# ossamaAhmed/blackbox_mpc

Measured on AMD Instinct MI355X. Metric: MPC control-steps/sec (agent-control-steps; Pendulum true model, CEM N=500 H=30), higher is better.
Workload: dtype f32; 1 GPU; BASELINE cfg2: Pendulum-v0 true dynamics, CEM, num_agents=1/GPU, N=500, H=30, 5 iters, k=50, closed loop (the model is the environment); parallelism=single GPU

## Files before the change

### blackbox_mpc_amd/csrc/bbmpc.hip

```cpp
#include "engine.hpp"
#include "abi_util.hpp"
#include "engine_util.hpp"
#include "kernels_corr.hpp"
#include "kernels_elite_carry.hpp"

#include <math.h>
#include <stdio.h>
#include <stdlib.h>
#include <atomic>
#include <functional>
#include <chrono>
#include <mutex>
#include <set>
#include <thread>
#include <utility>

namespace bbmpc {

static std::mutex g_engines_mu;
static std::set<Engine*> g_engines;
static std::atomic<int> g_resident_handles{0};
void note_resident_handle() { g_resident_handles.fetch_add(1, std::memory_order_relaxed); }

void stop_foreign_residents(Engine* self) {
// ... 128 lines not shown
        throw HipError(BBMPC_E_NO_DEVICE, "no HIP device available: this library has no CPU fallback");
    if (c.device >= 0) {
        REQUIRE(c.device < ndev, BBMPC_E_NO_DEVICE, "bbmpc_config.device out of range");
        HIP_CHECK(hipSetDevice(c.device));
    }
    HIP_CHECK(hipGetDevice(&device));
    HIP_CHECK(hipDeviceGetAttribute(&cu_count, hipDeviceAttributeMultiprocessorCount, device));
    {
        int least = 0, greatest = 0;
        HIP_CHECK(hipDeviceGetStreamPriorityRange(&least, &greatest));
        if (!(own_stream = masked_stream_from_env("BBMPC_STREAM_CUS", cu_count)))
            HIP_CHECK(hipStreamCreateWithPriority(&own_stream, hipStreamNonBlocking, greatest));
    }
    stream = own_stream;
    init_tnq_table();

    if (const char* fm = getenv("BBMPC_FUSED")) fused_mode = atoi(fm);
    {
        auto flag = [](const char* n) { return getenv(n) != nullptr; };
        auto ival = [](const char* n, int dflt) { const char* v = getenv(n); return v ? atoi(v) : dflt; };
        sw.cma_svd_v1 = flag("BBMPC_CMA_SVD_V1"); sw.cma_svd_rounds = flag("BBMPC_CMA_SVD_ROUNDS");
        sw.cma_svd_general = flag("BBMPC_CMA_SVD_GENERAL");
        sw.cma_svd_gram = flag("BBMPC_CMA_SVD_GRAM");
        sw.cma_coop = flag("BBMPC_CMA_COOP"); sw.cma_nb = ival("BBMPC_CMA_NB", 0);
        sw.cma_eigh = ival("BBMPC_CMA_EIGH", 1); sw.cma_eigh_fail = flag("BBMPC_CMA_EIGH_FAIL");
        sw.cma_fused = flag("BBMPC_CMA_FUSED");
        sw.mlp_generic = flag("BBMPC_MLP_GENERIC");
        { const int b = ival("BBMPC_MLP_BF16", 0); sw.mlp_bf16 = (b == 1 || b == 3) ? b : 0; }
        sw.mlp_pair = ival("BBMPC_MLP_PAIR", -1); sw.mlp_q4 = ival("BBMPC_MLP_Q4", -1); sw.mlp_q4s = ival("BBMPC_MLP_Q4S", ival("BBMPC_MLP_Q4R", 1)); sw.mlp_w4 = ival("BBMPC_MLP_W4", 1); sw.pi2_skip_init = ival("BBMPC_PI2_SKIP_INIT", 1); sw.step_graph = ival("BBMPC_STEP_GRAPH", 1); sw.cma_small3 = ival("BBMPC_CMA_SMALL3", 1);
        sw.refit_wgs = ival("BBMPC_REFIT_WGS", 0);
        sw.mlp_wave = ival("BBMPC_MLP_WAVE", 1);
        sw.linger_us = std::max(0, ival("BBMPC_LINGER_US", 200));
        linger_test_quit = ival("BBMPC_LINGER_TEST_QUIT", 0) - 1;
        sw.balance = ival("BBMPC_BALANCE", 0);
        sw.ilp = ival("BBMPC_ILP", 1) == 2 ? 2 : 1;
        sw.refit_v1 = flag("BBMPC_REFIT_V1");
        sw.zero_copy = !flag("BBMPC_NO_ZERO_COPY");
        sw.host_poll = !flag("BBMPC_NO_HOST_POLL");
        sw.mlp_no_half_tail = flag("BBMPC_MLP_NO_HALF_TAIL");
        sw.dbg = flag("BBMPC_DBG");
        sw.prof_reward_mlp = flag("BBMPC_PROF_REWARD_MLP");
        user_stepwise_only = flag("BBMPC_USER_STEPWISE");
        if (c.optimizer != BBMPC_OPT_NONE) {
            ps_loopback = auto_split > 1 ? auto_split : ival("BBMPC_POPSHARD_LOOPBACK", 0);
            ps_force = flag("BBMPC_POPSHARD_FORCE");
        }
    }
    HU = H * U;
    Nst = ((std::max(N, 1) + 63) / 64) * 64;
    rec = U + S + 1;
    lo.assign(c.action_low, c.action_low + U);
    hi.assign(c.action_high, c.action_high + U);
    upload(d_lo, lo);
    upload(d_hi, hi);
    d_state.alloc((size_t)A * S);
    d_record.alloc((size_t)A * rec);
    d_action.alloc((size_t)A * U);
    d_action.zero(stream);
    if (c.optimizer != BBMPC_OPT_NONE) {
        std::vector<float> m((size_t)A * HU), v((size_t)A * HU);
        for (int i = 0; i < A * HU; ++i) {
            const int u = i % U;
            m[i] = (lo[u] + hi[u]) / 2.0f;
            const float d = lo[u] - hi[u];
            v[i] = (d * d) / 16.0f;
        }
// ... 45 lines not shown
    }
    if (pf_stream) {
        (void)hipStreamSynchronize(pf_stream);
        (void)hipStreamDestroy(pf_stream);
        for (int b = 0; b < 2; ++b)
            if (pf_done[b]) (void)hipEventDestroy(pf_done[b]);
        if (pf_free) (void)hipEventDestroy(pf_free);
    }
    for (auto e : ev_pool) (void)hipEventDestroy(e);
    user_reward.release();
    user_dynamics.release();
    user_rollout.release();
    user_xform.release();
    user_fwd_xform.release();
    user_xform_rollout.release();
    if (h_pin) (void)hipHostFree(h_pin);
    for (auto*& hs : h_record_stage) { if (hs) (void)hipHostFree(hs); hs = nullptr; }
    if (host_done) (void)hipHostFree(host_done);
    if (host_count) (void)hipFree(host_count);
    if (own_stream) (void)hipStreamDestroy(own_stream);
}

void Engine::settle() {
    if (settle_hook) settle_hook(this);
    resident_stop();
    if (lazy_sync) {
        lazy_sync = false;
        HIP_CHECK(hipStreamSynchronize(stream));
    }
}

static void resident_unpublish(Engine* e);

bool Engine::resident_step(const float* state, int add_noise, uint32_t seq) {
    {
        bool all_gone = true;
        for (int a = 0; a < A && all_gone; ++a) all_gone = *(volatile const uint32_t*)gone_host(a) != 0u;
        if (all_gone) {
            resident_unpublish(this);
            resident_alive = false;
            return false;
        }
    }
    const uint32_t step = step_counter;
    const int64_t c = (int64_t)step / std::max(pf_steps, 1);
    const int pb = (int)(c & 1), nb = pb ^ 1;
    if (pf_mode != 1 || pf_chunk[pb] != c) { resident_stop(); return false; }
    if (!pf_waited[pb]) {
        if (hipEventQuery(pf_done[pb]) != hipSuccess) { resident_stop(); return false; }
        pf_waited[pb] = true; pf_inflight[pb] = false;
    }
    const float* inj = d_noise_pf[pb].p + (size_t)((int64_t)step - c * pf_steps) * pf_step_floats;
    ++step_counter;
    const uint64_t ip = (uint64_t)(uintptr_t)inj;
    for (int a = 0; a < A; ++a) {
        volatile uint32_t* m = mbox_host(a);
        uint32_t sw3[3];
        memcpy(sw3, state + (size_t)a * 3, 12);
        const uint32_t tag = seq & 0xffffu;
        const uint16_t half[13] = {(uint16_t)step, (uint16_t)(step >> 16), (uint16_t)(add_noise != 0),
                                   (uint16_t)ip, (uint16_t)(ip >> 16), (uint16_t)(ip >> 32), (uint16_t)(ip >> 48),
                                   (uint16_t)sw3[0], (uint16_t)(sw3[0] >> 16), (uint16_t)sw3[1], (uint16_t)(sw3[1] >> 16),
                                   (uint16_t)sw3[2], (uint16_t)(sw3[2] >> 16)};
        for (int i = 0; i < 13; ++i) m[i] = ((uint32_t)half[i] << 16) | tag;
        m[15] = seq;
    }
    std::atomic_thread_fence(std::memory_order_release);
    if (pf_chunk[nb] != c + 1) {
        launch_noise_fill(c + 1, nb, pf_stream);
        HIP_CHECK(hipEventRecord(pf_done[nb], pf_stream));
        pf_chunk[nb] = c + 1; pf_waited[nb] = false; pf_inflight[nb] = true;
    }
    if (in_flight_hook && !in_flight_called) { in_flight_called = true; in_flight_hook(this); }
    const auto t0 = std::chrono::steady_clock::now();
    bool all = true;
    for (int a = 0; a < A; ++a) {
        volatile const uint32_t* ack = ack_host(a);
        volatile const uint32_t* gone = gone_host(a);
        uint32_t spins = 0;
        for (;;) {
            if (*ack == seq) break;
            if (*gone != 0u) { all = false; break; }
            if ((++spins & 0xfff) == 0 && std::chrono::steady_clock::now() - t0 > std::chrono::seconds(2)) { all = false; break; }
        }
    }
    if (all) return true;
    resident_stop();
    int missing = 0;
    int32_t* amap = amap_host();
    for (int a = 0; a < A; ++a)
        if (*(volatile const uint32_t*)ack_host(a) != seq) amap[missing++] = a;
    if (missing == 0) return true;
    --step_counter;
    subset_n = missing < A ? missing : 0;
    return false;
}

static void resident_unpublish(Engine* e) {
    if (e->mbox_pub.load(std::memory_order_relaxed)) {
        e->mbox_pub.store(nullptr, std::memory_order_release);
        g_resident_handles.fetch_sub(1, std::memory_order_relaxed);
    }
}

void Engine::resident_stop() {
    if (!resident_alive) return;
    resident_unpublish(this);
    for (int a = 0; a < A; ++a) mbox_host(a)[15] = 0xffffffffu;
    std::atomic_thread_fence(std::memory_order_release);
    resident_alive = false;
    HIP_CHECK(hipStreamSynchronize(stream));
}

float* Engine::pinned(size_t count) {
    if (count > h_pin_n) {
        invalidate_step_graph();
        if (h_pin) (void)hipHostFree(h_pin);
        h_pin = nullptr;
        h_pin_n = 0;
        HIP_CHECK(hipHostMalloc((void**)&h_pin, count * sizeof(float), hipHostMallocCoherent | hipHostMallocMapped));
        h_pin_n = count;
        HIP_CHECK(hipHostGetDevicePointer((void**)&h_pin_dev, h_pin, 0));
    }
    return h_pin;
// ... 1223 lines not shown

}

static const float* optimize_host(bbmpc::Engine& e, const float* state, int32_t noise, float* action, float* next_state, float* reward) {
    using namespace bbmpc;
    const size_t ns = (size_t)e.A * e.S, nr = (size_t)e.A * e.rec;
    float* pin = e.pinned(ns + nr);
    memcpy(pin, state, ns * 4);
    bool published = false;
    bool handled_resident = false;
    const bool fused_step = e.sw.zero_copy && (e.use_fused() || e.use_fused_pso());
    const bool mlp_tail = e.sw.zero_copy && !fused_step && e.cfg.optimizer != BBMPC_OPT_NONE;
    if (fused_step || mlp_tail) {
        float* dpin = e.h_pin_dev;
        if (e.sw.host_poll && !e.trace_on) {
            if (!e.host_done) {
                HIP_CHECK(hipHostMalloc((void**)&e.host_done, (size_t)e.sync_lines() * 64, hipHostMallocCoherent | hipHostMallocMapped));
                memset(e.host_done, 0, (size_t)e.sync_lines() * 64);
                HIP_CHECK(hipHostGetDevicePointer((void**)&e.host_done_dev, e.host_done, 0));
                HIP_CHECK(hipMalloc((void**)&e.host_count, 8));
                HIP_CHECK(hipMemset(e.host_count, 0, 8));
            }
            if (++e.host_seq == 0) e.host_seq = 1;
            e.tail_flag = e.host_done_dev;
            e.tail_count = e.host_count;
            e.tail_value = e.host_seq;
            e.tail_attached = false;
        }
        const bool linger_ok = fused_step && e.tail_flag != nullptr && e.sw.linger_us > 0 && e.A <= Engine::kLingerMaxAgents && e.use_fused() &&
                               !e.profiling && e.tail_event == nullptr &&
                               e.stream == e.own_stream;
        bool handled = false;
        if (e.resident_alive) {
            if (linger_ok) handled = e.resident_step(pin, noise, e.host_seq);
            else e.resident_stop();
        }
        if (handled) ++e.calls_resident; else ++e.calls_launched;
        if (handled) {
            published = true;
            handled_resident = true;
            e.tail_flag = nullptr;
        } else
        try {
            e.linger_launch = linger_ok && e.subset_n == 0;
            if (fused_step) {
                e.optimize_dev(dpin, noise, dpin + ns, nullptr);
            } else {
                const bool stage = (e.cfg.optimizer == BBMPC_OPT_CEM || e.cfg.optimizer == BBMPC_OPT_PI2) && !e.pop_sharded() &&
                                   !e.user_path() && !e.value_on();
                const bool graph_ok = e.sw.step_graph && stage && e.cfg.dynamics == BBMPC_DYN_MLP && e.tail_flag != nullptr &&
                                      e.tail_event == nullptr && !e.profiling && !e.trace_on && !e.particles_on() && !e.corr_on() && !e.carry_on() && e.stream == e.own_stream && !e.any_injected();
                const uint64_t sig = ((uint64_t)e.mutations << 8) | (uint64_t)(noise ? 1 : 0) | 2u;
                bool replayed = false;
                if (graph_ok && e.step_graph && e.step_graph_sig == sig) {
                    replayed = true;
                } else if (graph_ok && e.step_graph_warm >= 3 && e.step_warm_sig == sig) {
                    if (e.step_graph) { (void)hipGraphExecDestroy(e.step_graph); e.step_graph = nullptr; }
                    if (!e.step_words) {
                        HIP_CHECK(hipHostMalloc((void**)&e.step_words, 64, 0));
                        memset(e.step_words, 0, 64);
                        HIP_CHECK(hipMalloc((void**)&e.step_words_dev, 64));
                        HIP_CHECK(hipMemset(e.step_words_dev, 0, 64));
                        e.step_mirror[0] = e.step_mirror[1] = 0xFFFFFFFFu;
                    }
                    const uint32_t saved_step = e.step_counter;
                    hipGraph_t g = nullptr;
                    bool ok = hipStreamBeginCapture(e.stream, hipStreamCaptureModeThreadLocal) == hipSuccess;
// ... 36 lines not shown
                e.optimize_dev(e.d_state.p, noise, dpin + ns, nullptr);
                if (e.stage_state_src) {
                    e.stage_state_src = nullptr;
                    throw HipError(BBMPC_E_HIP, "internal: the control step did not stage its state");
                }
                if (graph_ok && e.last_step_steady && e.step_warm_sig == sig) ++e.step_graph_warm;
                else { e.step_graph_warm = (graph_ok && e.last_step_steady) ? 1 : 0; e.step_warm_sig = sig; }
                }
            }
            e.linger_launch = false;
            published = e.tail_flag != nullptr && e.tail_attached;
            e.tail_flag = nullptr;
        } catch (...) {
            e.linger_launch = false;
            e.tail_flag = nullptr;
            e.subset_n = 0;
            throw;
        }
    } else {
        ++e.calls_launched;
        HIP_CHECK(hipMemcpyAsync(e.d_state.p, pin, ns * 4, hipMemcpyHostToDevice, e.stream));
        e.optimize_dev(e.d_state.p, noise, e.d_record.p, nullptr);
        HIP_CHECK(hipMemcpyAsync(pin + ns, e.d_record.p, nr * 4, hipMemcpyDeviceToHost, e.stream));
    }
    if (e.in_flight_hook && !e.in_flight_called) { e.in_flight_called = true; e.in_flight_hook(&e); }
    if (handled_resident) {
        std::atomic_thread_fence(std::memory_order_acquire);
        e.lazy_sync = true;
    } else if (published && e.resident_alive) {
        const uint32_t want = e.host_seq;
        const auto t0 = std::chrono::steady_clock::now();
        for (int a = 0; a < e.A; ++a) {
            volatile const uint32_t* f = e.ack_host(a);
            uint32_t spins = 0;
            while (*f != want) {
                if ((++spins & 0xfff) == 0 && std::chrono::steady_clock::now() - t0 > std::chrono::seconds(2)) {
                    e.resident_stop();
                    if (*f != want) throw HipError(BBMPC_E_HIP, "bbmpc_optimize: the control step finished without publishing its records");
                }
            }
        }
        std::atomic_thread_fence(std::memory_order_acquire);
        e.lazy_sync = true;
    } else if (published) {
        volatile const uint32_t* f = e.host_done;
        const uint32_t want = e.host_seq;
        const auto t0 = std::chrono::steady_clock::now();
        uint32_t spins = 0;
        while (*f != want) {
            if ((++spins & 0xfff) == 0 && std::chrono::steady_clock::now() - t0 > std::chrono::seconds(2)) {
                HIP_CHECK(hipStreamSynchronize(e.stream));
                if (*f != want) throw HipError(BBMPC_E_HIP, "bbmpc_optimize: the control step finished without publishing its records");
                break;
            }
        }
        std::atomic_thread_fence(std::memory_order_acquire);
        e.lazy_sync = true;
    } else {
        HIP_CHECK(hipStreamSynchronize(e.stream));
        e.lazy_sync = false;
    }
    const float* r = pin + ns;
    for (int a = 0; a < e.A; ++a) {
        if (action) memcpy(action + (size_t)a * e.U, r + (size_t)a * e.rec, e.U * 4);
        if (next_state) memcpy(next_state + (size_t)a * e.S, r + (size_t)a * e.rec + e.U, e.S * 4);
        if (reward) reward[a] = r[(size_t)a * e.rec + e.U + e.S];
    }
    return r;
}

extern "C" {
// ... 552 lines not shown
```

### blackbox_mpc_amd/csrc/bbmpc_fused.hip

```cpp
#define BBMPC_TU_FUSED
#include "engine.hpp"
#include "engine_util.hpp"

#include <atomic>
#include <chrono>

namespace bbmpc {

void bbmpc_tu_fused_upload_tnq(const float2* table) { tnq_upload(table); }

bool Engine::use_fused() const {
    if (cfg.dynamics != BBMPC_DYN_PENDULUM || cfg.reward != BBMPC_REW_PENDULUM) return false;
    if (pop_sharded()) return false;
    if (particles_on()) return false;
    if (corr_on()) return false;
    if (carry_on()) return false;
    if (cfg.optimizer == BBMPC_OPT_SPSA) {
        if (iters > FUSED_MAX_SPSA_ITERS) return false;
    } else if (cfg.optimizer != BBMPC_OPT_RANDOM_SEARCH && cfg.optimizer != BBMPC_OPT_CEM && cfg.optimizer != BBMPC_OPT_PI2) {
        return false;
    }
    if (fused_mode == 0) return false;
    if (fused_mode == 1) return true;
    return (long)N <= 2048 || A >= 64;
}

static void note_inst(Engine& e, int opt, bool samples_lds, bool fastm, int inj, int ilp, bool linger) {
    snprintf(e.dominant_inst, sizeof(e.dominant_inst), "k_fused_pendulum<%d, %s, %s, %d, %d, %s>", opt, samples_lds ? "true" : "false",
             fastm ? "true" : "false", inj, ilp, linger ? "true" : "false");
}

template <int OPT, bool FASTM, int INJ, int ILP>
static void launch_fused4(Engine& e, FusedArgs& fa, int threads, size_t lds_base, size_t lds_samples) {
#ifdef BBMPC_KERNEL_DBG
    const size_t limit = 158 * 1024;
#else
    const size_t limit = 160 * 1024;
#endif
    if (lds_base + lds_samples <= limit) {
        fa.test_quit_agent = -1;
        if constexpr (INJ == 2 && FASTM && ILP == 1) {
            if (e.linger_launch && e.subset_n == 0 && fa.done_flag && e.tail_event == nullptr) {
                auto fl = k_fused_pendulum<OPT, true, FASTM, INJ, ILP, true>;
                note_inst(e, OPT, true, FASTM, INJ, ILP, true);
                ensure_max_lds((const void*)fl, (int)limit);
                for (int a = 0; a < e.A; ++a) {
                    volatile uint32_t* m = e.mbox_host(a);
                    for (int i = 0; i < 13; ++i) m[i] = fa.done_value & 0xffffu;
                    m[15] = fa.done_value;
                    *(volatile uint32_t*)e.gone_host(a) = 0u;
                }
                std::atomic_thread_fence(std::memory_order_release);
                fa.done_flag = e.sync_dev(e.ack_host(0));
                fa.mbox = e.sync_dev(e.mbox_host(0));
                fa.gone = e.sync_dev(e.gone_host(0));
                fa.linger_ticks = (unsigned)e.sw.linger_us * 100u;
                fa.test_quit_agent = e.linger_test_quit;
                hipLaunchKernelGGL(fl, dim3(e.A), dim3(threads), lds_base + lds_samples, e.stream, fa);
                HIP_CHECK(hipGetLastError());
                e.resident_alive = true;
                if (!e.mbox_pub.load(std::memory_order_relaxed)) {
                    e.mbox_pub_agents = e.A;
                    e.mbox_pub.store(e.mbox_host(0), std::memory_order_release);
                    note_resident_handle();
                }
                return;
            }
        }
        if (e.subset_n > 0) {
            auto fs = k_fused_pendulum<OPT, true, FASTM, INJ, ILP>;
            note_inst(e, OPT, true, FASTM, INJ, ILP, false);
            ensure_max_lds((const void*)fs, (int)limit);
            fa.amap = reinterpret_cast<const int*>(e.sync_dev(e.amap_host()));
            hipLaunchKernelGGL(fs, dim3(e.subset_n), dim3(threads), lds_base + lds_samples, e.stream, fa);
            HIP_CHECK(hipGetLastError());
            e.subset_n = 0;
            return;
        }
        auto fn = k_fused_pendulum<OPT, true, FASTM, INJ, ILP>;
        note_inst(e, OPT, true, FASTM, INJ, ILP, false);
        ensure_max_lds((const void*)fn, (int)limit);
// ... 76 lines not shown
    fa.inj_expl = injected(BBMPC_NOISE_EXPLORATION);
    if (cfg.optimizer == BBMPC_OPT_SPSA) {
        const float big_a = (float)iters / 10.0f;
        for (int it = 0; it < iters && it < FUSED_MAX_SPSA_ITERS; ++it) {
            const float tf = (float)it;
            fa.spsa_ak[it] = cfg.spsa_a / (float)pow((double)((tf + 1.0f) + big_a), (double)cfg.spsa_alpha);
            fa.spsa_ck[it] = cfg.spsa_c / (float)pow((double)(tf + 1.0f), (double)cfg.spsa_gamma);
        }
    }
    fa.record = d_record_out;
    fa.next_state = d_next_out;
    if (trace_on) {
        ensure_trace();
        fa.t_rewards = t_rewards.p; fa.t_mean = t_mean.p; fa.t_var = t_var.p; fa.t_elites = t_elites.p; fa.t_samples = t_samples.p;
        if (cfg.optimizer == BBMPC_OPT_SPSA) {
            if (!t_rewards2.p) t_rewards2.alloc((size_t)A * Nst * std::max(iters, 1));
            fa.t_rewards2 = t_rewards2.p;
        }
    }
#ifdef BBMPC_KERNEL_DBG
    static long long* dbg_buf = nullptr;
    if (sw.dbg) {
        if (!dbg_buf) {
            HIP_CHECK(hipHostMalloc((void**)&dbg_buf, 64 * 8, hipHostMallocDefault));
            memset(dbg_buf, 0, 64 * 8);
        }
        if (dbg_buf[42]) {
            const long long* d = dbg_buf;
            fprintf(stderr, "[dbg] last resident pass, 10ns units rel. to its start:");
            for (int i = 0; i <= 1 + iters * 4; ++i) fprintf(stderr, " %lld", d[i] - d[0]);
            fprintf(stderr, "\n[dbg] iter0 per-wave rollout end:");
            for (int i = 24; i < 32; ++i) fprintf(stderr, " %lld", d[i] - d[0]);
            fprintf(stderr, "\n[dbg] request accepted %lld  first model step %lld  completion stored %lld\n", d[42] - d[0], d[44] - d[0], d[43] - d[0]);
            dbg_buf[42] = 0;
        }
        fa.dbg = dbg_buf;
    }
#endif
    fa.key = key(step);
    const int pf_nit = cfg.optimizer == BBMPC_OPT_RANDOM_SEARCH ? 1 : iters;
    if (pf_mode < 0) {
        const char* ev = getenv("BBMPC_NOISE_PREFETCH");
        pf_step_floats = (size_t)pf_nit * A * Nst * ((HU + 3) / 4) * 4;
        const size_t budget = (size_t)128 << 20;
        pf_steps = pf_step_floats ? (int)std::min<size_t>(8, budget / (pf_step_floats * 4)) : 0;
        pf_mode = ((ev ? atoi(ev) != 0 : true) && pf_steps >= 1 && U == 1) ? 1 : 0;
        if (pf_mode) {
            {
                int least = 0, greatest = 0;
                HIP_CHECK(hipDeviceGetStreamPriorityRange(&least, &greatest));
                HIP_CHECK(hipStreamCreateWithPriority(&pf_stream, hipStreamNonBlocking, greatest));
            }
            HIP_CHECK(hipEventCreateWithFlags(&pf_free, hipEventDisableTiming));
            for (int b = 0; b < 2; ++b) {
                d_noise_pf[b].alloc(pf_step_floats * pf_steps);
                HIP_CHECK(hipEventCreateWithFlags(&pf_done[b], hipEventDisableTiming));
            }
        }
    }
    const bool use_pf = pf_mode == 1 && fa.inj == nullptr && pf_nit > 0;
    if (use_pf) {
        const int64_t c = (int64_t)step / pf_steps;
        const int pb = (int)(c & 1), nb = pb ^ 1;
        if (pf_chunk[pb] != c) {
            if (pf_inflight[pb]) HIP_CHECK(hipStreamWaitEvent(stream, pf_done[pb], 0));
            launch_noise_fill(c, pb, stream);
// ... 117 lines not shown
```

### blackbox_mpc_amd/csrc/engine.hpp

```cpp
#pragma once
#include <hip/hip_ext.h>
#include <hip/hip_runtime.h>
#include <stdint.h>
#include <string.h>

#include <algorithm>
#include <atomic>
#include <map>
#include <stdexcept>
#include <string>
#include <vector>

#include "../../include/bbmpc.h"
#include "comm.hpp"
#include "kernels_cma.hpp"
#include "kernels_eigh.hpp"
#include "kernels_eigh_small.hpp"
#include "kernels_fused.hpp"
#include "kernels_fused_cma.hpp"
#include "kernels_fused_pso.hpp"
#include "kernels_mlp.hpp"
#include "kernels_mlp_xform.hpp"
#include "kernels_mlp_q4s.hpp"
#include "kernels_mlp_w4.hpp"
#include "kernels_mlp_wave.hpp"
#include "kernels_opt.hpp"
#include "kernels_refit.hpp"
#include "kernels_reward_mlp.hpp"
#include "kernels_rollout.hpp"
#include "kernels_tail.hpp"
#include "kernels_user.hpp"

namespace bbmpc {

struct ParticleArgs;
struct TrajParticleArgs;

struct HipError : std::runtime_error {
    int code;
    HipError(int c, const std::string& m) : std::runtime_error(m), code(c) {}
};

#define HIP_CHECK(expr)                                                                          \
    do {                                                                                         \
        hipError_t _e = (expr);                                                                  \
        if (_e != hipSuccess)                                                                    \
            throw HipError(BBMPC_E_HIP, std::string(#expr) + " failed: " + hipGetErrorString(_e) + \
// ... 151 lines not shown
    float* gather_deferred_dst[RecordComm::kSlots] = {nullptr, nullptr};
    void (*settle_hook)(Engine*) = nullptr;
    void (*in_flight_hook)(Engine*) = nullptr;
    bool in_flight_called = false;
    hipEvent_t tail_event = nullptr;
    bool tail_attached = false;
    uint32_t* tail_flag = nullptr;
    uint32_t tail_value = 0;
    uint32_t* tail_count = nullptr;
    uint32_t* host_done = nullptr;
    uint32_t* host_done_dev = nullptr;
    uint32_t* host_count = nullptr;
    uint32_t host_seq = 0;
    bool lazy_sync = false;
    void settle();
    const float* stage_state_src = nullptr;
    bool linger_launch = false;
    bool resident_alive = false;
    static constexpr int kLingerMaxAgents = 64;
    int sync_lines() const {
        const int al = std::max(1, std::min(A, kLingerMaxAgents));
        return 1 + 3 * al + (al + 15) / 16;
    }
    uint32_t* ack_host(int a) { return host_done + 16 * (1 + a); }
    uint32_t* mbox_host(int a) { return host_done + 16 * (1 + std::min(A, kLingerMaxAgents) + a); }
    uint32_t* gone_host(int a) { return host_done + 16 * (1 + 2 * std::min(A, kLingerMaxAgents) + a); }
    int32_t* amap_host() { return reinterpret_cast<int32_t*>(host_done + 16 * (1 + 3 * std::min(A, kLingerMaxAgents))); }
    uint32_t* sync_dev(const void* host_ptr) { return host_done_dev + (reinterpret_cast<const uint32_t*>(host_ptr) - host_done); }
    std::atomic<uint32_t*> mbox_pub{nullptr};
    int mbox_pub_agents = 0;
    int subset_n = 0;
    int linger_test_quit = -1;
    int64_t calls_resident = 0, calls_launched = 0;
    bool resident_step(const float* state, int add_noise, uint32_t seq);
    void resident_stop();
    hipStream_t pf_stream = nullptr;
    hipEvent_t pf_done[2] = {nullptr, nullptr}, pf_free = nullptr;
    int64_t pf_chunk[2] = {-1, -1};
    bool pf_waited[2] = {false, false}, pf_inflight[2] = {false, false};
    int pf_steps = 0;
    size_t pf_step_floats = 0;
    int pf_mode = -1;
    void launch_noise_fill(int64_t chunk, int buf, hipStream_t on);
    std::vector<hipEvent_t> ev_pool;
    size_t ev_used = 0;
    const char* dominant_kernel = "k_rollout_pendulum";
    char dominant_inst[128] = "";

    explicit Engine(const bbmpc_config& c);
    ~Engine();

    RngKey key(uint32_t step) const {
        RngKey kk;
        kk.k0 = (uint32_t)(cfg.seed & 0xffffffffu);
        kk.k1 = (uint32_t)(cfg.seed >> 32);
        kk.step = step;
        kk.q_per_agent = (uint32_t)((HU + 3) / 4);
        kk.step_src = step_capturing ? step_words_dev : nullptr;
        return kk;
    }
    bool fix(uint32_t bit) const { return (cfg.quirks & bit) != 0; }
    UserFunction user_reward, user_dynamics, user_rollout;
    bool user_rollout_stale = true;
    bool user_stepwise_only = false;
    void rollout_user_fused(int mode, bool pen, RolloutArgs& ra);
    void rollout_mlp_user_reward(int mode, bool pen, RolloutArgs& ra);
    DevBuf<float> u_traj;
// ... 209 lines not shown
```

### blackbox_mpc_amd/csrc/kernels_fused.hpp

```cpp
#pragma once
#include <type_traits>

#include "kernels_opt.hpp"
#include "kernels_refit.hpp"
#include "kernels_rollout.hpp"
#include "topk.hpp"

namespace bbmpc {

constexpr int FOPT_RS = 1;
constexpr int FOPT_CEM = 2;
constexpr int FOPT_PI2 = 3;
constexpr int FOPT_SPSA = 4;
constexpr int FUSED_MAX_SPSA_ITERS = 16;

struct FusedArgs {
    int N, A, H, U, HU, Nst, k, iters;
    int agent_offset;
    int fix_q1, fix_q7, add_noise;
    int warm_start;
    int balance;
    unsigned* done_flag;
    unsigned* done_count;
    unsigned done_value;
// ... 96 lines not shown
                mean[tid] = m_keep;
                var[tid] = v_keep;
                sigma[tid] = (OPT == FOPT_CEM && p.warm_start) ? cem_sigma(m_keep, v_keep, lo, hi) : s_keep;
            }
        } else {
            for (int j = tid; j < p.HU; j += nthr) {
                const float m = p.prev_mean[a * p.HU + j];
                const float v = p.var0[a * p.HU + j];
                const float sg = (OPT == FOPT_CEM) ? cem_sigma(m, v, lo, hi) : ((OPT == FOPT_SPSA) ? 0.0f : sqrtf(v));
                mean[j] = m;
                var[j] = v;
                sigma[j] = sg;
                if (keep_init) { m_keep = m; v_keep = v; s_keep = sg; }
            }
        }
    };
    typedef float pfvec4 __attribute__((ext_vector_type(4)));
    typedef const __attribute__((address_space(1))) pfvec4* pfvec4p;
    [[maybe_unused]] pfvec4 pf0 = {0.0f, 0.0f, 0.0f, 0.0f}, pf1 = {0.0f, 0.0f, 0.0f, 0.0f};
    [[maybe_unused]] auto prefetch_first = [&](const float* base, int it_n) {
        if constexpr (INJ == 2) {
            const int Q = (p.HU + 3) >> 2;
            if (tid < p.N) {
                const pfvec4p q = (pfvec4p)(reinterpret_cast<const float4*>(base) + noise_block_index(it_n, p.A, a, p.Nst, tid, Q));
                pf0 = q[0];
                if (OPT != FOPT_SPSA) pf1 = q[min(1, Q - 1)];
            }
        }
    };
    dist_init(false);
    __syncthreads();
    float s0 = red[60], s1 = red[61], s2 = red[62];
    if (p.iters > 0) prefetch_first(inj_s, 0);
    for (;;) {

        float action0 = (OPT == FOPT_RS) ? 0.0f : mean[0];

        BB_DBG(0);
#ifdef BBMPC_KERNEL_DBG
        if (p.dbg && tid == 0 && a == 0) dbg_lds[40] = (long long)clock64();
#endif
        for (int it = 0; it < p.iters; ++it) {
            BB_DBG(1 + it * 4);
            const float* inj = (INJ == 1) ? inj_s + ((size_t)it * p.A + a) * p.HU * p.Nst : nullptr;
            const int nblk = p.H >> 2, rem = p.H & 3;
            const uint32_t rstream = (OPT == FOPT_RS) ? 2u : 1u;
            auto with_q1 = [&](auto&& body) {
                if constexpr (FASTM) {
                    if (p.fix_q1 != 0) { body(std::true_type{}); return; }
                }
                body(std::false_type{});
            };
            if constexpr (OPT == FOPT_SPSA) {
                const float ck = p.spsa_ck[it];
                const int nb4 = (p.H + 3) >> 2;
                with_q1([&](auto Q1c) {
                constexpr bool Q1 = decltype(Q1c)::value;
                for (int n = tid; n < p.N; n += nthr) {
                    Roller<FASTM> rp, rm;
                    rp.init(p.fix_q1 != 0, s0, s1, s2);
                    rm.init(p.fix_q1 != 0, s0, s1, s2);
                    float tp = 0.0f, tm = 0.0f, pp = 0.0f, pm = 0.0f;
                    typedef float gvec4s __attribute__((ext_vector_type(4)));
                    typedef const __attribute__((address_space(1))) gvec4s* gvec4sp;
                    [[maybe_unused]] gvec4sp mine4 = nullptr;
                    [[maybe_unused]] gvec4s cur4 = {1.0f, 1.0f, 1.0f, 1.0f};
// ... 344 lines not shown
                }
                __syncthreads();
                action0 = mean[0];
            } else {
                float bv = -INFINITY;
                int bi = 0x7fffffff;
                for (int n = tid; n < p.N; n += nthr) {
                    const float v = rew[n];
                    if (v > bv || (v == bv && n < bi)) { bv = v; bi = n; }
                }
                wave_argmax(bv, bi);
                int* redi = (int*)(red + 32);
                if ((tid & 63) == 0) { red[tid >> 6] = bv; redi[tid >> 6] = bi; }
                __syncthreads();
                bv = ((tid & 63) < nw) ? red[tid & 63] : -INFINITY;
                bi = ((tid & 63) < nw) ? redi[tid & 63] : 0x7fffffff;
                wave_argmax(bv, bi);
                if (bi == 0x7fffffff) bi = 0;
                action0 = samp[bi];
                if (p.t_elites && tid == 0) p.t_elites[a] = bi;
                __syncthreads();
            }
            if (p.t_mean && OPT != FOPT_RS)
                for (int j = tid; j < p.HU; j += nthr) {
                    p.t_mean[((size_t)it * p.A + a) * p.HU + j] = mean[j];
                    p.t_var[((size_t)it * p.A + a) * p.HU + j] = var[j];
                }
        }

        BB_DBG(1 + p.iters * 4);
#ifdef BBMPC_KERNEL_DBG
        if (p.dbg && tid == 0 && a == 0) dbg_lds[41] = (long long)clock64();
#endif
        if (OPT != FOPT_RS) {
            for (int j = tid; j < p.HU; j += nthr) {
                p.mean_out[a * p.HU + j] = mean[j];
                p.var_out[a * p.HU + j] = var[j];
                if (OPT == FOPT_PI2 || OPT == FOPT_SPSA) {
                    const int js = (j + 1 < p.HU) ? j + 1 : p.HU - 1;
                    const float pm = mean[js];
                    p.prev_mean[a * p.HU + j] = pm;
                    if (keep_init) m_keep = pm;
                } else if (p.warm_start) {
                    const float pm = mean[j];
                    p.prev_mean[a * p.HU + j] = pm;
                    if (keep_init) m_keep = pm;
                }
            }
        }

        if (tid == 0) {
            FinalArgs fa;
            fa.A = p.A; fa.U = 1; fa.S = 3;
            fa.agent_offset = p.agent_offset;
            fa.fix_q1 = p.fix_q1; fa.fix_q7 = p.fix_q7;
            fa.add_noise = add_noise_s;
            fa.lo = p.lo; fa.hi = p.hi;
            fa.inj = p.inj_expl;
            fa.key = key_s;
            fa.key.q_per_agent = 1;
            float s[3] = {s0, s1, s2};
            float act[1];
            act[0] = exploration_action(fa, a, 0, action0);
            const float r = model.step(s, act);
            float* rec = p.record + (size_t)a * 5;
            rec[0] = act[0];
            rec[1] = s[0];
            rec[2] = s[1];
            rec[3] = s[2];
            rec[4] = r;
            if (p.next_state) {
                p.next_state[a * 3 + 0] = s[0];
                p.next_state[a * 3 + 1] = s[1];
                p.next_state[a * 3 + 2] = s[2];
            }
            if constexpr (LINGER) publish_records_done(p.done_flag + a * 16, nullptr, done_value_s, 1u);
            else publish_records_done(p.done_flag, p.done_count, done_value_s, gridDim.x);
            BB_DBG(43);
#ifdef BBMPC_KERNEL_DBG
            if (p.dbg && a == 0) for (int i = 0; i < 48; ++i) p.dbg[i] = dbg_lds[i];
#endif
        }
        if constexpr (!LINGER) {
            break;
        } else {
            unsigned* mb = (unsigned*)ekeys;
            __syncthreads();
            dist_init(keep_init);
            [[maybe_unused]] const float* inj_pred = nullptr;
            if constexpr (INJ == 2) {
                if (p.pf_step_floats)
                    for (int b = 0; b < 2; ++b)
                        if (inj_s >= p.pf_buf[b] && inj_s + 2 * p.pf_step_floats <= p.pf_buf[b] + p.pf_chunk_floats) inj_pred = inj_s + p.pf_step_floats;
                if (inj_pred && p.iters > 0) prefetch_first(inj_pred, 0);
            }
            if (tid < 64) {
                const long long t0 = (long long)wall_clock64();
                const unsigned want = done_value_s + 1u;
                unsigned w = 0u;
                bool quit = false;
                for (;;) {
                    w = (tid < 16) ? __hip_atomic_load(p.mbox + a * 16 + tid, __ATOMIC_RELAXED, __HIP_MEMORY_SCOPE_SYSTEM) : 0u;
                    const bool mine = tid < 13 ? (w & 0xffffu) == (want & 0xffffu) : (tid == 15 ? w == want : true);
                    const unsigned w15 = __builtin_amdgcn_readlane(w, 15);
                    if (__builtin_amdgcn_ballot_w64(mine) == ~0ull) break;
                    if (w15 == 0xffffffffu || (long long)wall_clock64() - t0 > (long long)p.linger_ticks || a == p.test_quit_agent || (p.test_quit_agent >= 999 && a >= p.test_quit_agent - 999)) { quit = true; break; }
                }
                if (tid < 16) mb[tid] = (quit && tid == 15) ? 0xffffffffu : w;
                BB_DBG(42);
            }
            __syncthreads();
            if (mb[15] == 0xffffffffu) {
                if (tid == 0) __hip_atomic_store(p.gone + a * 16, done_value_s, __ATOMIC_RELEASE, __HIP_MEMORY_SCOPE_SYSTEM);
                return;
            }
// ... 15 lines not shown
```

### blackbox_mpc_amd/csrc/kernels_refit.hpp

```cpp
#pragma once
#include <hip/hip_runtime.h>
#include <math.h>
#include "models.hpp"
#include "rng.hpp"
#include "topk.hpp"

namespace bbmpc {

constexpr int REFIT_THREADS = 1024;

#define BB_DPP_QUAD_XOR1 0xB1
#define BB_DPP_QUAD_XOR2 0x4E
#define BB_DPP_ROW_HALF_MIRROR 0x141
#define BB_DPP_ROW_MIRROR 0x140
#define BB_DPP_ROW_SHR(n) (0x110 + (n))

template <int CTRL>
__device__ __forceinline__ float dpp_f(float v) {
    return __int_as_float(__builtin_amdgcn_update_dpp(0, __float_as_int(v), CTRL, 0xf, 0xf, false));
}
template <int CTRL>
__device__ __forceinline__ int dpp_i(int v) {
    return __builtin_amdgcn_update_dpp(0, v, CTRL, 0xf, 0xf, false);
}
// ... 277 lines not shown
}

static __global__ void k_argmax_merge(RefitArgs p, const float* all, int G) {
    const int a = blockIdx.x, lane = threadIdx.x;
    const size_t pw = (size_t)p.A * (p.U + 2);
    int br = 0, bi = 0x7fffffff;
    float bv = -INFINITY;
    for (int r = 0; r < G; ++r) {
        const float* e = all + pw * r + (size_t)a * (p.U + 2);
        const float v = e[0];
        const int idx = __float_as_int(e[1]);
        if (v > bv || (v == bv && idx < bi) || bi == 0x7fffffff) { bv = v; bi = idx; br = r; }
    }
    const float* src = all + pw * br + (size_t)a * (p.U + 2) + 2;
    if (lane == 0 && p.elites) p.elites[a] = bi;
    if (lane < p.U) p.action[a * p.U + lane] = src[lane];
}

struct FinalArgs {
    int A, U, S;
    int agent_offset;
    int fix_q1, fix_q7;
    int add_noise;
    const float* state;
    const float* action;
    const float* lo;
    const float* hi;
    const float* inj;
    float* record;
    float* next_state;
    RngKey key;
};

__device__ __forceinline__ float exploration_action(const FinalArgs& p, int a, int u, float act) {
    if (!p.add_noise) return act;
    float xi;
    if (p.inj) xi = p.inj[a * p.U + u];
    else {
        U4 b = rng_block(rng_key_now(p.key), 10u , 0u, 0u, (uint32_t)(p.agent_offset + a), (uint32_t)u);
        xi = word_to_trunc_normal(pick_word(b, (uint32_t)u));
    }
    const float lo = p.lo[u], hi = p.hi[u];
    const float d = lo - hi;
    const float var = (d * d) / 16.0f * 0.05f;
    const float mean = p.fix_q7 ? 0.0f : (hi + lo) / 2.0f;
    const float noise = xi * sqrtf(var) + mean;
    return clipf(act + noise, lo, hi);
}

__device__ __forceinline__ void finalize_pendulum_agent(const FinalArgs& p, int a, float action_in) {
    const PendulumModel model{p.fix_q1 != 0};
    float s[3] = {p.state[a * 3 + 0], p.state[a * 3 + 1], p.state[a * 3 + 2]};
    float act[1];
    act[0] = exploration_action(p, a, 0, action_in);
    const float r = model.step(s, act);
    float* rec = p.record + (size_t)a * (1 + 3 + 1);
    rec[0] = act[0];
    rec[1] = s[0];
    rec[2] = s[1];
    rec[3] = s[2];
    rec[4] = r;
    if (p.next_state) {
        p.next_state[a * 3 + 0] = s[0];
        p.next_state[a * 3 + 1] = s[1];
        p.next_state[a * 3 + 2] = s[2];
    }
}
__device__ __forceinline__ void publish_records_done(unsigned* flag, unsigned* count, unsigned value, unsigned nwg) {
    if (!flag) return;
    if (nwg == 1u) {
        __hip_atomic_store(flag, value, __ATOMIC_RELEASE, __HIP_MEMORY_SCOPE_SYSTEM);
        return;
    }
    const unsigned old = __hip_atomic_fetch_add(count, 1u, __ATOMIC_RELEASE, __HIP_MEMORY_SCOPE_AGENT);
    if (old == nwg - 1u) {
        __builtin_amdgcn_fence(__ATOMIC_ACQUIRE, "agent");
        __hip_atomic_store(count, 0u, __ATOMIC_RELAXED, __HIP_MEMORY_SCOPE_AGENT);
        __hip_atomic_store(flag, value, __ATOMIC_RELEASE, __HIP_MEMORY_SCOPE_SYSTEM);
    }
}
// ... 12 lines not shown
```

Baseline: 29980 control-steps/s.

## Publish pendulum step record inside the completion line and move tail earlier

The resident (lingering) pendulum kernel now packs the 5-float step record into the 64-byte completion line. Each 32-bit word carries 16 record bits plus a 16-bit sequence tag, written by 16 lanes with system-scope atomic stores. The host decodes the record straight from that line while polling, avoiding a separate record write and its fence-ordered publish. The tail (noise, model step, publish) also runs before the mean/carry stores, to cut latency to the host. This adds tag-based torn-read detection and an encoding constraint that the record is exactly 5 floats.

Result: faster. 30530 control-steps/s, median of 6 (+1.8%).

```diff
diff --git a/blackbox_mpc_amd/csrc/bbmpc.hip b/blackbox_mpc_amd/csrc/bbmpc.hip
--- a/blackbox_mpc_amd/csrc/bbmpc.hip
+++ b/blackbox_mpc_amd/csrc/bbmpc.hip
@@ -184,6 +184,7 @@
         sw.mlp_wave = ival("BBMPC_MLP_WAVE", 1);
         sw.linger_us = std::max(0, ival("BBMPC_LINGER_US", 200));
         linger_test_quit = ival("BBMPC_LINGER_TEST_QUIT", 0) - 1;
+        host_seq = (uint32_t)ival("BBMPC_TEST_HOST_SEQ", 0);
         sw.balance = ival("BBMPC_BALANCE", 0);
         sw.ilp = ival("BBMPC_ILP", 1) == 2 ? 2 : 1;
         sw.refit_v1 = flag("BBMPC_REFIT_V1");
@@ -295,7 +296,7 @@
 
 static void resident_unpublish(Engine* e);
 
-bool Engine::resident_step(const float* state, int add_noise, uint32_t seq) {
+bool Engine::resident_step(const float* state, int add_noise, uint32_t seq, float* records) {
     {
         bool all_gone = true;
         for (int a = 0; a < A && all_gone; ++a) all_gone = *(volatile const uint32_t*)gone_host(a) != 0u;
@@ -342,7 +343,7 @@
         volatile const uint32_t* gone = gone_host(a);
         uint32_t spins = 0;
         for (;;) {
-            if (*ack == seq) break;
+            if (completion_line_decode(ack, seq, records + (size_t)a * kCompletionRecordFloats)) break;
             if (*gone != 0u) { all = false; break; }
             if ((++spins & 0xfff) == 0 && std::chrono::steady_clock::now() - t0 > std::chrono::seconds(2)) { all = false; break; }
         }
@@ -352,7 +353,7 @@
     int missing = 0;
     int32_t* amap = amap_host();
     for (int a = 0; a < A; ++a)
-        if (*(volatile const uint32_t*)ack_host(a) != seq) amap[missing++] = a;
+        if (!completion_line_decode(ack_host(a), seq, records + (size_t)a * kCompletionRecordFloats)) amap[missing++] = a;
     if (missing == 0) return true;
     --step_counter;
     subset_n = missing < A ? missing : 0;
@@ -1642,7 +1643,7 @@
                                e.stream == e.own_stream;
         bool handled = false;
         if (e.resident_alive) {
-            if (linger_ok) handled = e.resident_step(pin, noise, e.host_seq);
+            if (linger_ok) handled = e.resident_step(pin, noise, e.host_seq, pin + ns);
             else e.resident_stop();
         }
         if (handled) ++e.calls_resident; else ++e.calls_launched;
@@ -1745,11 +1746,12 @@
         const auto t0 = std::chrono::steady_clock::now();
         for (int a = 0; a < e.A; ++a) {
             volatile const uint32_t* f = e.ack_host(a);
+            float* rec_a = pin + ns + (size_t)a * kCompletionRecordFloats;
             uint32_t spins = 0;
-            while (*f != want) {
+            while (!completion_line_decode(f, want, rec_a)) {
                 if ((++spins & 0xfff) == 0 && std::chrono::steady_clock::now() - t0 > std::chrono::seconds(2)) {
                     e.resident_stop();
-                    if (*f != want) throw HipError(BBMPC_E_HIP, "bbmpc_optimize: the control step finished without publishing its records");
+                    if (!completion_line_decode(f, want, rec_a)) throw HipError(BBMPC_E_HIP, "bbmpc_optimize: the control step finished without publishing its records");
                 }
             }
         }
diff --git a/blackbox_mpc_amd/csrc/bbmpc_fused.hip b/blackbox_mpc_amd/csrc/bbmpc_fused.hip
--- a/blackbox_mpc_amd/csrc/bbmpc_fused.hip
+++ b/blackbox_mpc_amd/csrc/bbmpc_fused.hip
@@ -44,9 +44,11 @@
                 auto fl = k_fused_pendulum<OPT, true, FASTM, INJ, ILP, true>;
                 note_inst(e, OPT, true, FASTM, INJ, ILP, true);
                 ensure_max_lds((const void*)fl, (int)limit);
+                if (e.rec != kCompletionRecordFloats) throw HipError(BBMPC_E_HIP, "internal: the resident pendulum kernel's record is not 5 floats");
                 for (int a = 0; a < e.A; ++a) {
                     volatile uint32_t* m = e.mbox_host(a);
-                    for (int i = 0; i < 13; ++i) m[i] = fa.done_value & 0xffffu;
+                    volatile uint32_t* cl = e.ack_host(a);
+                    for (int i = 0; i < 16; ++i) cl[i] = (fa.done_value - 1u) & 0xffffu;                    for (int i = 0; i < 13; ++i) m[i] = fa.done_value & 0xffffu;
                     m[15] = fa.done_value;
                     *(volatile uint32_t*)e.gone_host(a) = 0u;
                 }
@@ -189,6 +191,9 @@
             fprintf(stderr, "\n[dbg] iter0 per-wave rollout end:");
             for (int i = 24; i < 32; ++i) fprintf(stderr, " %lld", d[i] - d[0]);
             fprintf(stderr, "\n[dbg] request accepted %lld  first model step %lld  completion stored %lld\n", d[42] - d[0], d[44] - d[0], d[43] - d[0]);
+            const long long sel = d[iters > 0 ? 4 * iters : 0];
+            fprintf(stderr, "[dbg] tail rel. to the last selection: tail start %lld  noise applied %lld  model step %lld  record stored %lld  published %lld  last barrier %lld  carry stored %lld\n",
+                    d[38] - sel, d[35] - sel, d[36] - sel, d[37] - sel, d[43] - sel, d[1 + iters * 4] - sel, d[34] - sel);
             dbg_buf[42] = 0;
         }
         fa.dbg = dbg_buf;
diff --git a/blackbox_mpc_amd/csrc/completion_line.hpp b/blackbox_mpc_amd/csrc/completion_line.hpp
--- /dev/null
+++ b/blackbox_mpc_amd/csrc/completion_line.hpp
@@ -0,0 +1,35 @@
+#pragma once
+#include <cstdint>
+#include <cstring>
+
+namespace bbmpc {
+
+constexpr int kCompletionRecordFloats = 5;
+
+inline bool completion_line_decode(const volatile uint32_t* line, uint32_t seq, float* rec) {
+    if (line[15] != seq) return false;
+    uint32_t w[2 * kCompletionRecordFloats];
+    for (int i = 0; i < 2 * kCompletionRecordFloats; ++i) w[i] = line[i];
+    const uint32_t tag = seq & 0xffffu;
+    for (int i = 0; i < 2 * kCompletionRecordFloats; ++i)
+        if ((w[i] & 0xffffu) != tag) return false;
+    for (int f = 0; f < kCompletionRecordFloats; ++f) {
+        const uint32_t bits = (w[2 * f] >> 16) | (w[2 * f + 1] & 0xffff0000u);
+        memcpy(rec + f, &bits, 4);
+    }
+    return true;
+}
+
+inline void completion_line_encode(uint32_t* line, uint32_t seq, const float* rec) {
+    const uint32_t tag = seq & 0xffffu;
+    for (int f = 0; f < kCompletionRecordFloats; ++f) {
+        uint32_t bits;
+        memcpy(&bits, rec + f, 4);
+        line[2 * f] = (bits << 16) | tag;
+        line[2 * f + 1] = (bits & 0xffff0000u) | tag;
+    }
+    for (int i = 2 * kCompletionRecordFloats; i < 15; ++i) line[i] = tag;
+    line[15] = seq;
+}
+
+}
diff --git a/blackbox_mpc_amd/csrc/engine.hpp b/blackbox_mpc_amd/csrc/engine.hpp
--- a/blackbox_mpc_amd/csrc/engine.hpp
+++ b/blackbox_mpc_amd/csrc/engine.hpp
@@ -13,6 +13,7 @@
 
 #include "../../include/bbmpc.h"
 #include "comm.hpp"
+#include "completion_line.hpp"
 #include "kernels_cma.hpp"
 #include "kernels_eigh.hpp"
 #include "kernels_eigh_small.hpp"
@@ -230,7 +231,7 @@
     int subset_n = 0;
     int linger_test_quit = -1;
     int64_t calls_resident = 0, calls_launched = 0;
-    bool resident_step(const float* state, int add_noise, uint32_t seq);
+    bool resident_step(const float* state, int add_noise, uint32_t seq, float* records);
     void resident_stop();
     hipStream_t pf_stream = nullptr;
     hipEvent_t pf_done[2] = {nullptr, nullptr}, pf_free = nullptr;
diff --git a/blackbox_mpc_amd/csrc/kernels_fused.hpp b/blackbox_mpc_amd/csrc/kernels_fused.hpp
--- a/blackbox_mpc_amd/csrc/kernels_fused.hpp
+++ b/blackbox_mpc_amd/csrc/kernels_fused.hpp
@@ -152,6 +152,53 @@
     __syncthreads();
     float s0 = red[60], s1 = red[61], s2 = red[62];
     if (p.iters > 0) prefetch_first(inj_s, 0);
+    auto noise_term = [&]() {
+        FinalArgs fa;
+        fa.A = p.A; fa.U = 1; fa.S = 3;
+        fa.agent_offset = p.agent_offset;
+        fa.fix_q1 = p.fix_q1; fa.fix_q7 = p.fix_q7;
+        fa.add_noise = add_noise_s;
+        fa.lo = p.lo; fa.hi = p.hi;
+        fa.inj = p.inj_expl;
+        fa.key = key_s;
+        fa.key.q_per_agent = 1;
+        return exploration_noise(fa, a, 0, lo, hi);
+    };
+    const bool tail_lanes = LINGER ? tid < 64 : tid == 0;
+    auto tail = [&](float act_in) {
+        BB_DBG(38);
+        float s[3] = {s0, s1, s2};
+        float act[1];
+        act[0] = add_noise_s ? exploration_apply(act_in, noise_term(), lo, hi) : act_in;
+        BB_DBG(35);
+        const float r = model.step(s, act);
+        BB_DBG(36);
+        if constexpr (LINGER) {
+            const unsigned tag = done_value_s & 0xffffu;
+            const float f = tid < 2 ? act[0] : (tid < 4 ? s[0] : (tid < 6 ? s[1] : (tid < 8 ? s[2] : r)));
+            const unsigned bits = __float_as_uint(f);
+            unsigned w = ((tid & 1) ? (bits & 0xffff0000u) : (bits << 16)) | tag;
+            if (tid >= 10) w = tag;
+            if (tid == 15) w = done_value_s;
+            if (tid < 16) __hip_atomic_store(p.done_flag + a * 16 + tid, w, __ATOMIC_RELAXED, __HIP_MEMORY_SCOPE_SYSTEM);
+            BB_DBG(37);
+        } else {
+            float* rec = p.record + (size_t)a * 5;
+            rec[0] = act[0];
+            rec[1] = s[0];
+            rec[2] = s[1];
+            rec[3] = s[2];
+            rec[4] = r;
+            if (p.next_state) {
+                p.next_state[a * 3 + 0] = s[0];
+                p.next_state[a * 3 + 1] = s[1];
+                p.next_state[a * 3 + 2] = s[2];
+            }
+            BB_DBG(37);
+            publish_records_done(p.done_flag, p.done_count, done_value_s, gridDim.x);
+        }
+        BB_DBG(43);
+    };
     for (;;) {
 
         float action0 = (OPT == FOPT_RS) ? 0.0f : mean[0];
@@ -562,6 +609,7 @@
 #ifdef BBMPC_KERNEL_DBG
         if (p.dbg && tid == 0 && a == 0) dbg_lds[41] = (long long)clock64();
 #endif
+        if (tail_lanes) tail(action0);
         if (OPT != FOPT_RS) {
             for (int j = tid; j < p.HU; j += nthr) {
                 p.mean_out[a * p.HU + j] = mean[j];
@@ -578,39 +626,10 @@
                 }
             }
         }
-
-        if (tid == 0) {
-            FinalArgs fa;
-            fa.A = p.A; fa.U = 1; fa.S = 3;
-            fa.agent_offset = p.agent_offset;
-            fa.fix_q1 = p.fix_q1; fa.fix_q7 = p.fix_q7;
-            fa.add_noise = add_noise_s;
-            fa.lo = p.lo; fa.hi = p.hi;
-            fa.inj = p.inj_expl;
-            fa.key = key_s;
-            fa.key.q_per_agent = 1;
-            float s[3] = {s0, s1, s2};
-            float act[1];
-            act[0] = exploration_action(fa, a, 0, action0);
-            const float r = model.step(s, act);
-            float* rec = p.record + (size_t)a * 5;
-            rec[0] = act[0];
-            rec[1] = s[0];
-            rec[2] = s[1];
-            rec[3] = s[2];
-            rec[4] = r;
-            if (p.next_state) {
-                p.next_state[a * 3 + 0] = s[0];
-                p.next_state[a * 3 + 1] = s[1];
-                p.next_state[a * 3 + 2] = s[2];
-            }
-            if constexpr (LINGER) publish_records_done(p.done_flag + a * 16, nullptr, done_value_s, 1u);
-            else publish_records_done(p.done_flag, p.done_count, done_value_s, gridDim.x);
-            BB_DBG(43);
-#ifdef BBMPC_KERNEL_DBG
-            if (p.dbg && a == 0) for (int i = 0; i < 48; ++i) p.dbg[i] = dbg_lds[i];
-#endif
-        }
+        BB_DBG(34);
+#ifdef BBMPC_KERNEL_DBG
+        if (p.dbg && a == 0 && tid == 0) for (int i = 0; i < 48; ++i) p.dbg[i] = dbg_lds[i];
+#endif
         if constexpr (!LINGER) {
             break;
         } else {
diff --git a/blackbox_mpc_amd/csrc/kernels_refit.hpp b/blackbox_mpc_amd/csrc/kernels_refit.hpp
--- a/blackbox_mpc_amd/csrc/kernels_refit.hpp
+++ b/blackbox_mpc_amd/csrc/kernels_refit.hpp
@@ -333,20 +333,25 @@
     RngKey key;
 };
 
-__device__ __forceinline__ float exploration_action(const FinalArgs& p, int a, int u, float act) {
-    if (!p.add_noise) return act;
+__device__ __forceinline__ float exploration_noise(const FinalArgs& p, int a, int u, float lo, float hi) {
     float xi;
     if (p.inj) xi = p.inj[a * p.U + u];
     else {
         U4 b = rng_block(rng_key_now(p.key), 10u , 0u, 0u, (uint32_t)(p.agent_offset + a), (uint32_t)u);
         xi = word_to_trunc_normal(pick_word(b, (uint32_t)u));
     }
-    const float lo = p.lo[u], hi = p.hi[u];
     const float d = lo - hi;
     const float var = (d * d) / 16.0f * 0.05f;
     const float mean = p.fix_q7 ? 0.0f : (hi + lo) / 2.0f;
-    const float noise = xi * sqrtf(var) + mean;
+    return xi * sqrtf(var) + mean;
+}
+__device__ __forceinline__ float exploration_apply(float act, float noise, float lo, float hi) {
     return clipf(act + noise, lo, hi);
+}
+__device__ __forceinline__ float exploration_action(const FinalArgs& p, int a, int u, float act) {
+    if (!p.add_noise) return act;
+    const float lo = p.lo[u], hi = p.hi[u];
+    return exploration_apply(act, exploration_noise(p, a, u, lo, hi), lo, hi);
 }
 
 __device__ __forceinline__ void finalize_pendulum_agent(const FinalArgs& p, int a, float action_in) {
```
